# hasindu2008/cornetto

Hardware: AMD Instinct MI355X
Metric: Gbases/s scanned (telowin+sdust+boringbits) (higher is better)
Workload: dtype u8/u16 integer

## Files before the change

cornetto_amd/csrc/cov.hip:

```cpp
#include <algorithm>
#include <cmath>

#include "common.hpp"
#include "scan.hpp"
#include "tiles.hpp"
#include "ivlmerge.hpp"
#include "internal.hpp"

namespace {

constexpr int CB_THREADS = 256;
#ifndef CN_CB_PARTS
#define CN_CB_PARTS 2
#endif
constexpr int CB_PARTS = CN_CB_PARTS;
constexpr int CB_MAX_INC_LDS = 128;

struct CbArgs {
    const uint16_t *depth, *mq;
    const int64_t *ctg_off;
    const int32_t *ctg_len;
    const int2 *tiles;
    int32_t inc, r;
    uint2 *pre;
    uint2 *head;
    int64_t n_tiles;
    const int4 *tmeta;
    uint2 *tile_tot32;
    ulonglong2 *tile_tot64;
};

typedef unsigned short cb_us2 __attribute__((ext_vector_type(2)));
__device__ __forceinline__ uint32_t add_u16x2(uint32_t acc, uint32_t pair)
{
    const cb_us2 ones = {1, 1};
    return __builtin_amdgcn_udot2(__builtin_bit_cast(cb_us2, pair), ones, acc, false);
}

typedef unsigned int cb_u4 __attribute__((ext_vector_type(4)));

template <bool STAGE, int INC, int NT = 1>
__global__ __launch_bounds__(CB_THREADS) void cov_blocks(CbArgs A)
{
    __builtin_amdgcn_s_setprio(CN_STREAM_PRIO);

    extern __shared__ __attribute__((aligned(16))) uint8_t smem[];
    __shared__ uint32_t wsum[2][CB_THREADS / 64];
    __shared__ unsigned long long wsum64[2][CB_THREADS / 64];

    const int t = threadIdx.x;
    const int inc = INC ? INC : A.inc, r = A.r;
    constexpr int PBc = CB_THREADS / CB_PARTS;
    constexpr int NVIc = INC ? (PBc * INC / 8 + CB_THREADS - 1) / CB_THREADS : 4;
    cb_u4 pre_all[NT][2][CB_PARTS][NVIc];
    if (STAGE && INC) {
#pragma unroll
        for (int ti = 0; ti < NT; ++ti) {
            const int64_t tix = (int64_t)blockIdx.x * NT + ti;
            if (tix >= A.n_tiles) continue;
            int2 tl;
            int ln;
            int64_t of;
            if (A.tmeta) {
                const int4 m0 = A.tmeta[2 * tix], m1 = A.tmeta[2 * tix + 1];
                tl = make_int2(m0.x, m0.y); ln = m0.z; of = (int64_t)(((unsigned long long)(uint32_t)m1.y << 32) | (uint32_t)m1.x);
            } else {
                tl = A.tiles[tix]; ln = A.ctg_len[tl.x]; of = A.ctg_off[tl.x];
            }
            const int64_t e0l = (int64_t)tl.y * inc;
            const int nvec = PBc * inc / 8;
#pragma unroll
            for (int which = 0; which < 2; ++which)
#pragma unroll
                for (int part = 0; part < CB_PARTS; ++part) {
                    const int64_t pe0 = e0l + (int64_t)part * PBc * inc;
                    const int64_t left = ((int64_t)ln - pe0) * 2;
                    const uint32_t nrec = left <= 0 ? 0u : (uint32_t)(left < (int64_t)nvec * 16 ? (left + 15) & ~15LL : (int64_t)nvec * 16);
                    const __amdgpu_buffer_rsrc_t rs = __builtin_amdgcn_make_buffer_rsrc((void *)((which ? A.mq : A.depth) + of + pe0), 0, (int)nrec, 0x00020000);
#pragma unroll
                    for (int k = 0; k < NVIc; ++k) pre_all[ti][which][part][k] = __builtin_amdgcn_raw_buffer_load_b128(rs, (t + k * CB_THREADS) * 16, 0, 0);
                }
        }
    }
#pragma unroll
  for (int ti = 0; ti < NT; ++ti) {
    const int64_t tix = (int64_t)blockIdx.x * NT + ti;
    if (tix >= A.n_tiles) break;
    if (ti) __syncthreads();
    int2 tile;
    int len;
    int64_t off;
    if (A.tmeta) {
        const int4 m0 = A.tmeta[2 * tix], m1 = A.tmeta[2 * tix + 1];
        tile = make_int2(m0.x, m0.y); len = m0.z; off = (int64_t)(((unsigned long long)(uint32_t)m1.y << 32) | (uint32_t)m1.x);
    } else {
        tile = A.tiles[tix]; len = A.ctg_len[tile.x]; off = A.ctg_off[tile.x];
    }
    const int64_t e0 = (int64_t)tile.y * inc;
    const int64_t p0 = e0 + (int64_t)t * inc;

    uint32_t fd = 0, fq = 0, hd = 0, hq = 0;
    unsigned long long xd = 0, xq = 0;
    if (STAGE) {
        uint16_t *sv = reinterpret_cast<uint16_t *>(smem);
        constexpr int PB = CB_THREADS / CB_PARTS;
        const int nvec = PB * inc / 8;
        const int base = (t % PB) * inc;
        const int nval = p0 >= len ? 0 : (int)(len - p0 < inc ? len - p0 : inc);
        const int nh = r < nval ? r : nval;
        constexpr int NVI = NVIc;
        auto &pre = pre_all[ti];
#pragma unroll
        for (int which = 0; which < 2; ++which) {
#pragma unroll
            for (int part = 0; part < CB_PARTS; ++part) {
                const int64_t pe0 = e0 + (int64_t)part * PB * inc;
                const int64_t left = ((int64_t)len - pe0) * 2;
                const uint32_t nrec = left <= 0 ? 0u : (uint32_t)(left < (int64_t)nvec * 16 ? (left + 15) & ~15LL : (int64_t)nvec * 16);
                const __amdgpu_buffer_rsrc_t rs = __builtin_amdgcn_make_buffer_rsrc((void *)((which ? A.mq : A.depth) + off + pe0), 0, (int)nrec, 0x00020000);
                if (which | part) __syncthreads();
                constexpr int NV = 4;
                if (INC) {
#pragma unroll
                    for (int k = 0; k < NVI; ++k) {
                        const int v = t + k * CB_THREADS;
                        if (v < nvec) reinterpret_cast<cb_u4 *>(sv)[v] = pre[which][part][k];
                    }
                } else
                for (int v0 = t; v0 < nvec; v0 += NV * CB_THREADS) {
                    cb_u4 a[NV];
#pragma unroll
                    for (int k = 0; k < NV; ++k) a[k] = __builtin_amdgcn_raw_buffer_load_b128(rs, (v0 + k * CB_THREADS) * 16, 0, 0);
#pragma unroll
                    for (int k = 0; k < NV; ++k) {
                        const int v = v0 + k * CB_THREADS;
                        if (v < nvec) reinterpret_cast<cb_u4 *>(sv)[v] = a[k];
                    }
                }
                __syncthreads();
                if (t / PB == part) {
                    uint32_t f = 0, hh = 0;
                    if (INC && (INC & 1) == 0 && nval == inc) {
                        const uint32_t *wd = reinterpret_cast<const uint32_t *>(sv + base);
#pragma unroll
                        for (int i = 0; i < (INC ? INC : 2) / 2; ++i) f = add_u16x2(f, wd[i]);
                    } else if (nval == inc && (inc & 1) == 0) {
                        const uint32_t *wd = reinterpret_cast<const uint32_t *>(sv + base);
                        for (int i = 0; i < inc / 2; ++i) f = add_u16x2(f, wd[i]);
                    } else {
#pragma clang loop vectorize(disable) unroll(disable)
                        for (int i = 0; i < nval; ++i) f += sv[base + i];
                    }
#pragma clang loop vectorize(disable) unroll(disable)
                    for (int i = 0; i < nh; ++i) hh += sv[base + i];
// ... 169 lines not shown
        if (k % 3 == 2 && k + 1 < NR) __builtin_amdgcn_sched_barrier(0);
    }

    if (lane == 0) {
        wsum[0][wv] = cd[NR];
        wsum[1][wv] = cq[NR];
    }
    __syncthreads();
    const bool front = (uint32_t)(lane & 3) < wv;
    const uint32_t wd = wsum[0][lane & 3], wq = wsum[1][lane & 3];
    uint32_t fd = front ? wd : 0u, fq = front ? wq : 0u;
    fd += (uint32_t)__builtin_amdgcn_update_dpp(0, (int)fd, 0xB1, 0xF, 0xF, true);
    fq += (uint32_t)__builtin_amdgcn_update_dpp(0, (int)fq, 0xB1, 0xF, 0xF, true);
    fd += (uint32_t)__builtin_amdgcn_update_dpp(0, (int)fd, 0x4E, 0xF, 0xF, true);
    fq += (uint32_t)__builtin_amdgcn_update_dpp(0, (int)fq, 0x4E, 0xF, 0xF, true);
    const __amdgpu_buffer_rsrc_t rso = __builtin_amdgcn_make_buffer_rsrc((void *)(A.pre + (size_t)tix * CB_THREADS + wv * 64), 0, 64 * (int)sizeof(uint2), 0x00020000);
#pragma unroll
    for (int k = 0; k < NR; ++k) {
        const cb_u2 o = {od[k] + fd + cd[k], oq[k] + fq + cq[k]};
        __builtin_amdgcn_raw_buffer_store_b64(o, rso, (int)ooff[k], 0, 0);
    }
    if (wv == CB_THREADS / 64 - 1 && lane == 0) {
        A.tile_tot32[tix] = make_uint2(cd[NR] + fd, cq[NR] + fq);
        ulonglong2 x;
        x.x = cd[NR] + fd;
        x.y = cq[NR] + fq;
        A.tile_tot64[tix] = x;
    }
}

__global__ __launch_bounds__(256) void cov_total64(const ulonglong2 *tot64, int64_t n, unsigned long long *grand )
{
    __shared__ unsigned long long sa[4], sb[4];
    unsigned long long a = 0, b = 0;
    for (int64_t i = (int64_t)blockIdx.x * 256 + threadIdx.x; i < n; i += (int64_t)gridDim.x * 256) {
        const ulonglong2 v = tot64[i];
        a += v.x;
        b += v.y;
    }
#pragma unroll
    for (int d = 32; d >= 1; d >>= 1) {
        a += ((unsigned long long)__shfl_xor((unsigned)(a >> 32), d) << 32) | __shfl_xor((unsigned)a, d);
        b += ((unsigned long long)__shfl_xor((unsigned)(b >> 32), d) << 32) | __shfl_xor((unsigned)b, d);
    }
    if ((threadIdx.x & 63) == 0) {
        sa[threadIdx.x >> 6] = a;
        sb[threadIdx.x >> 6] = b;
    }
    __syncthreads();
    if (threadIdx.x == 0) {
        atomicAdd(&grand[0], sa[0] + sa[1] + sa[2] + sa[3]);
        atomicAdd(&grand[1], sb[0] + sb[1] + sb[2] + sb[3]);
    }
}

struct CwArgs {
    const uint2 *pre, *head;
    const uint32_t *toff_d, *toff_q;
    const int64_t *blk_off;
    const int32_t *ctg_len;
    const int32_t *n_reg;
    const int2 *tiles;
    int32_t w, inc, q, r;
    uint32_t w_magic, w_shift;
    int32_t mode;
    int32_t lo, hi, edge, min_len;
    double low_mq;
    cornetto_reg_t *regs;
    cornetto_regrec_t *sel;
    cornetto_regpk_t *pk;
    uint2 *tile_res;
};

__device__ __forceinline__ uint2 cw_prefix(const CwArgs &A, int64_t x)
{
    const uint2 b = A.pre[x];
    return make_uint2(b.x + A.toff_d[x >> 8], b.y + A.toff_q[x >> 8]);
}

__global__ __launch_bounds__(256) void cov_windows(CwArgs A)
{
    __builtin_amdgcn_s_setprio(CN_STREAM_PRIO);

    __shared__ uint32_t wcnt[4];
    const int t = threadIdx.x;
    const int2 tile = A.tiles[blockIdx.x];
    const int ctg = tile.x;
    const int len = A.ctg_len[ctg];
    const int j = tile.y + t;
    bool valid = j < A.n_reg[ctg];
    int st = 0, end = 0, depth = 0, mq = 0;
    bool sel = false;
    if (valid) {
        st = j * A.inc;
        end = st + A.w;
        if (end > len) end = len;
        const int64_t a = A.blk_off[ctg] + j;
        uint32_t sd = 0, sq = 0;
        if (A.q > 0) {
            const uint2 hi = cw_prefix(A, a + A.q - 1);
            uint2 lo = make_uint2(0, 0);
            if (a > 0) lo = cw_prefix(A, a - 1);
            sd = hi.x - lo.x;
            sq = hi.y - lo.y;
        }
        if (A.r) {
            const uint2 hb = A.head[a + A.q];
            sd += hb.x;
            sq += hb.y;
        }
        if (end - st == A.w && A.w_magic && (int32_t)(sd | sq) >= 0) {
            depth = (int32_t)(__umulhi(sd, A.w_magic) >> A.w_shift);
            mq = (int32_t)(__umulhi(sq, A.w_magic) >> A.w_shift);
        } else {
            depth = (int32_t)sd / (end - st);
            mq = (int32_t)sq / (end - st);
        }
        if (A.mode == 0) {
            A.regs[j] = cornetto_reg_t{st, end, depth, mq};
        } else {
            bool fun = depth < A.lo || depth > A.hi;
            if (!fun && !(A.low_mq <= 1.0 && depth > 0 && mq >= depth)) fun = ((double)mq / (double)depth) < A.low_mq;
            if (A.mode == 1) sel = len >= A.min_len && fun;
            else sel = len > A.min_len && st > A.edge && end < len - A.edge && !fun;
        }
    }
    if (A.mode == 0) return;
    const unsigned long long bal = __ballot(sel);
    const int lane = t & 63, wv = t >> 6;
    if (lane == 0) wcnt[wv] = (uint32_t)__popcll(bal);
    __syncthreads();
    uint32_t pre = 0, tot = 0;
#pragma unroll
    for (int i = 0; i < 4; ++i) {
        if (i < wv) pre += wcnt[i];
        tot += wcnt[i];
    }
    if (t == 0) A.tile_res[blockIdx.x] = make_uint2(blockIdx.x * 256u, tot);
    if (sel) {
        const size_t idx = (size_t)blockIdx.x * 256u + pre + __popcll(bal & ((1ull << lane) - 1ull));
        if (A.pk) A.pk[idx] = cornetto_regpk_t{st, (uint16_t)depth, (uint16_t)mq};
        else A.sel[idx] = cornetto_regrec_t{ctg, st, end, depth, mq};
    }
}

__global__ void cov_ctg_first(const uint32_t *ooff, const int32_t *first_tile, int32_t n_ctg, uint32_t n_tiles, const unsigned long long *total, uint32_t *out)
{
    const int32_t i = (int32_t)(blockIdx.x * blockDim.x + threadIdx.x);
    if (i >= n_ctg) return;
    const uint32_t t = (uint32_t)first_tile[i];
    out[i] = t < n_tiles ? ooff[t] : (uint32_t)*total;
}

template <int INTS>
__global__ __launch_bounds__(256) void cov_order(const int32_t *raw, const uint2 *tres, const uint32_t *ooff, int64_t n_tiles, int32_t *dst, const unsigned long long *total,
                                                 uint32_t cap)
{
    const int64_t t = (int64_t)blockIdx.x * 4 + (threadIdx.x >> 6);
    if (t >= n_tiles) return;
    if (*total > cap) return;
    const uint2 r = tres[t];
    const int32_t *src = raw + (size_t)r.x * INTS;
    int32_t *d = dst + (size_t)ooff[t] * INTS;
    const uint32_t nint = r.y * (uint32_t)INTS;
    for (uint32_t i = threadIdx.x & 63; i < nint; i += 64) d[i] = src[i];
}

__global__ __launch_bounds__(256) void cov_order_expand(const cornetto_regpk_t *raw, const uint2 *tres, const uint32_t *ooff, int64_t n_tiles, cornetto_regrec_t *dst,
                                                        const unsigned long long *total, uint32_t cap, const int2 *tiles, const int32_t *ctg_len, int32_t w)
{
    const int64_t t = (int64_t)blockIdx.x * 4 + (threadIdx.x >> 6);
    if (t >= n_tiles) return;
    if (*total > cap) return;
    const uint2 r = tres[t];
    const int32_t ctg = tiles[t].x, len = ctg_len[ctg];
    const cornetto_regpk_t *src = raw + r.x;
    cornetto_regrec_t *d = dst + ooff[t];
    for (uint32_t i = threadIdx.x & 63; i < r.y; i += 64) {
        const cornetto_regpk_t p = src[i];
        const int64_t e = (int64_t)p.st + w;
        d[i] = cornetto_regrec_t{ctg, p.st, e > len ? len : (int32_t)e, (int32_t)p.depth, (int32_t)p.mq_depth};
    }
}

int32_t n_reg_host(int32_t length, int32_t w, int32_t inc)
{
    int32_t n = (length - w + inc - 1) / inc + 1;
    return n < 1 ? 1 : n;
}

int32_t regs_assert_host(int32_t length, int32_t w, int32_t inc)
{
    const int64_t st = (int64_t)(n_reg_host(length, w, inc) - 1) * inc;
    int64_t end = st + w;
    if (end > length) end = length;
    if (!(st < end)) return 353;
    return end == length ? 0 : 368;
}

}

extern "C" {

int32_t cornetto_n_reg(int32_t length, int32_t window_size, int32_t window_inc)
{
    if (window_inc <= 0) return 0;
    return n_reg_host(length, window_size, window_inc);
}

int32_t cornetto_regs_assert(int32_t length, int32_t window_size, int32_t window_inc)
{
    if (window_inc <= 0) return 353;
    return regs_assert_host(length, window_size, window_inc);
}

int32_t cornetto_cov_threshold(float factor, int32_t mean)
{
    return (int32_t)round(factor * mean);
}

int cornetto_cov_prepare(cornetto_accel_t *h, cornetto_cov_t *c, int32_t w, int32_t inc, uint64_t sums[3])
{
    if (!h || !c || !sums) return cn_fail(h, CORNETTO_E_ARG, "cov_prepare: bad argument");
    CN_HIP(h, hipSetDevice(h->device));
    cn_timing_begin(h);
    const int rc = cn_cov_prepare_impl(h, c, w, inc, sums);
    if (rc == CORNETTO_OK) cn_timing_end(h);
    return rc;
}

}

struct CwTileFill {
    int2 *out;
    __device__ void operator()(int64_t t, int ci, int64_t j) const { out[t] = make_int2(ci, (int)(j * 256)); }
};
struct CbTileFill {
    int2 *tiles;
    int4 *tmeta;
    const int32_t *len;
    const int64_t *off;
    __device__ void operator()(int64_t t, int ci, int64_t j) const
    {
        const int b = (int)(j * CB_THREADS);
        const unsigned long long o = (unsigned long long)off[ci];
        tiles[t] = make_int2(ci, b);
        tmeta[2 * t] = make_int4(ci, b, len[ci], 0);
        tmeta[2 * t + 1] = make_int4((int)(uint32_t)o, (int)(uint32_t)(o >> 32), 0, 0);
    }
};

int cn_cov_prepare_impl(cornetto_accel_t *h, cornetto_cov_t *c, int32_t w, int32_t inc, uint64_t sums[3])
{
    if (inc < 1) return cn_fail(h, CORNETTO_E_UNSUPPORTED, "cov_prepare: needs window_inc >= 1 (got -i %d: the reference divides by it)", inc);
    for (int32_t i = 0; i < c->n; ++i) {
        const int32_t line = c->len[i] < 1 ? 0 : regs_assert_host(c->len[i], w, inc);
        if (line)
            return cn_fail(h, CORNETTO_E_ASSERT, "src/boringbits_main.c:%d: get_regs: Assertion `%s' failed. (contig %d of length %d, -w %d -i %d)", line,
                           line == 353 ? "st<end" : "end == length", i, c->len[i], w, inc);
    }
    const int32_t q = w / inc, r = w % inc;
    sums[0] = sums[1] = 0;
    sums[2] = (uint64_t)c->total;
    CN_TRACE("cov_prepare: enter");
    if (c->w != w || c->inc != inc || !c->d_blk) {
        struct Invalidate {
            cornetto_cov_t *c;
            bool keep = false;
            ~Invalidate() { if (!keep) c->w = c->inc = -1; }
        } built{c};
        c->w = w;
        c->inc = inc;
        c->cw_mode = -1;
        c->blk_off.assign(c->n + 1, 0);
        c->n_reg.assign(c->n, 0);
        for (int32_t i = 0; i < c->n; ++i) {
            if (c->len[i] < 1) return cn_fail(h, CORNETTO_E_ARG, "cov_prepare: contig %d is empty (a bedgraph cannot produce that)", i);
            c->n_reg[i] = n_reg_host(c->len[i], w, inc);
            c->blk_off[i + 1] = c->blk_off[i] + cn_align_up((int64_t)c->n_reg[i] + q + 1, CB_THREADS);
        }
        c->n_blk = c->blk_off[c->n];
        const int64_t ntl = cntiles::prefix(h, c->cb_pref, c->n, [&](int32_t i) { return (c->blk_off[i + 1] - c->blk_off[i]) / CB_THREADS; });
        if (ntl < 0) return cn_fail(h, CORNETTO_E_NOMEM, "cov_prepare: device allocation failed");
        c->n_cb_tiles = ntl;
        if (c->d_blk) { (void)hipFree(c->d_blk); c->d_blk = nullptr; }
        if (c->d_blk_off) { (void)hipFree(c->d_blk_off); c->d_blk_off = nullptr; }
        if (c->d_cb_tiles) { (void)hipFree(c->d_cb_tiles); c->d_cb_tiles = nullptr; }
        if (c->d_cb_tmeta) { (void)hipFree(c->d_cb_tmeta); c->d_cb_tmeta = nullptr; }
        if (c->d_n_reg) { (void)hipFree(c->d_n_reg); c->d_n_reg = nullptr; }
        const size_t nt = (size_t)ntl;
        if (nt == 0) { built.keep = true; return CORNETTO_OK; }
        if (cn_obj_malloc(h, (void **)&c->d_blk, (size_t)c->n_blk * sizeof(uint4) + 2 * nt * sizeof(uint32_t)) != hipSuccess ||
            cn_obj_malloc(h, (void **)&c->d_blk_off, (size_t)(c->n + 1) * 8) != hipSuccess ||
            cn_obj_malloc(h, (void **)&c->d_cb_tiles, nt * sizeof(int2)) != hipSuccess ||
            cn_obj_malloc(h, (void **)&c->d_cb_tmeta, 2 * nt * sizeof(int4)) != hipSuccess ||
            cn_obj_malloc(h, (void **)&c->d_n_reg, (size_t)c->n * 4) != hipSuccess)
            return cn_fail(h, CORNETTO_E_NOMEM, "cov_prepare: device allocation failed");
        cntiles::fill<<<dim3((unsigned)((nt + 255) / 256)), dim3(256), 0, h->stream>>>(c->cb_pref.dev, c->n, ntl, CbTileFill{c->d_cb_tiles, c->d_cb_tmeta, c->d_len, c->d_off});
        CN_HIP(h, hipGetLastError());
        CN_HIP(h, hipMemcpyAsync(c->d_blk_off, c->blk_off.data(), (size_t)(c->n + 1) * 8, hipMemcpyHostToDevice, h->stream));
        CN_HIP(h, hipMemcpyAsync(c->d_n_reg, c->n_reg.data(), (size_t)c->n * 4, hipMemcpyHostToDevice, h->stream));
        built.keep = true;
    }
    CN_TRACE("cov_prepare: tables");
    const size_t nt = (size_t)c->n_cb_tiles;
    if (nt == 0) return CORNETTO_OK;
    uint2 *d_t32 = (uint2 *)cn_ws(h, WS_CB_T32, nt * sizeof(uint2));
    ulonglong2 *d_t64 = (ulonglong2 *)cn_ws(h, WS_CB_T64, nt * sizeof(ulonglong2));
    unsigned long long *d_grand = (unsigned long long *)cn_ws(h, WS_CB_GRAND, 16);
    unsigned long long *p_grand = (unsigned long long *)cn_pin(h, PIN_SMALL, 64);
    if (!d_t32 || !d_t64 || !d_grand || !p_grand) return cn_fail(h, CORNETTO_E_NOMEM, "cov_prepare: workspace allocation failed");
    uint2 *d_pre = reinterpret_cast<uint2 *>(c->d_blk), *d_head = d_pre + c->n_blk;
    uint32_t *d_toff_d = reinterpret_cast<uint32_t *>(d_head + c->n_blk), *d_toff_q = d_toff_d + nt;
    CN_TRACE("cov_prepare: workspaces");
    CN_HIP(h, hipMemsetAsync(d_grand, 0, 16, h->stream));
    static const int cb_tmeta = CN_DEV_INT("CORNETTO_COV_TMETA", 1);
    CbArgs A{c->d_depth, c->d_mq, c->d_off, c->d_len, c->d_cb_tiles, inc, r, d_pre, d_head, (int64_t)nt, cb_tmeta ? c->d_cb_tmeta : nullptr, d_t32, d_t64};
    if (inc <= CB_MAX_INC_LDS) {
        const size_t lds = (size_t)CB_THREADS / CB_PARTS * inc * sizeof(uint16_t);
        static_assert(CB_THREADS / CB_PARTS * 50 / 8 <= 4 * CB_THREADS, "cov_blocks<true, INC>: at most 4 vectors per thread and part");
        if (A.inc == 50 && r == 0 && A.tmeta && !CN_DEV_INT("CORNETTO_COV_BLOCKS_STAGE", 0)) {
            CN_LAUNCH(h, "cov_blocks", cov_blocks_scan<50><<<dim3((unsigned)nt), dim3(CB_THREADS), 0, h->stream>>>(A, CbsPattern<50>{}.masks()));
        } else if (A.inc == 50) {
            static const int cb_nt = CN_DEV_INT("CORNETTO_COV_TILES", 1);
            if (cb_nt == 2) {
                CN_HIP(h, hipFuncSetAttribute(reinterpret_cast<const void *>(&cov_blocks<true, 50, 2>), hipFuncAttributeMaxDynamicSharedMemorySize, (int)lds));
                CN_LAUNCH(h, "cov_blocks", cov_blocks<true, 50, 2><<<dim3((unsigned)((nt + 1) / 2)), dim3(CB_THREADS), lds, h->stream>>>(A));
            } else {
                CN_HIP(h, hipFuncSetAttribute(reinterpret_cast<const void *>(&cov_blocks<true, 50>), hipFuncAttributeMaxDynamicSharedMemorySize, (int)lds));
                CN_LAUNCH(h, "cov_blocks", cov_blocks<true, 50><<<dim3((unsigned)nt), dim3(CB_THREADS), lds, h->stream>>>(A));
            }
        } else {
            CN_HIP(h, hipFuncSetAttribute(reinterpret_cast<const void *>(&cov_blocks<true, 0>), hipFuncAttributeMaxDynamicSharedMemorySize, (int)lds));
            CN_LAUNCH(h, "cov_blocks", cov_blocks<true, 0><<<dim3((unsigned)nt), dim3(CB_THREADS), lds, h->stream>>>(A));
        }
    } else {
        CN_LAUNCH(h, "cov_blocks", cov_blocks<false, 0><<<dim3((unsigned)nt), dim3(CB_THREADS), 0, h->stream>>>(A));
    }
    {
        uint32_t *const outs[2] = {d_toff_d, d_toff_q};
        CN_TRY(cnscan::exclusive_u32_multi(h, "cov_tilescan", reinterpret_cast<const uint32_t *>(d_t32), (int64_t)nt, 2, 2, outs, nullptr));
    }
    const unsigned nb64 = (unsigned)std::min<size_t>(1024, (nt + 255) / 256);
    CN_LAUNCH(h, "cov_total64", cov_total64<<<dim3(nb64), dim3(256), 0, h->stream>>>(d_t64, (int64_t)nt, d_grand));
    CN_HIP(h, hipMemcpyAsync(p_grand, d_grand, 16, hipMemcpyDeviceToHost, h->stream));
    CN_TRACE("cov_prepare: queued");
    CN_HIP(h, hipStreamSynchronize(h->stream));
    CN_TRACE("cov_prepare: done");
    sums[0] = p_grand[0] - c->sum_corr[0];
    sums[1] = p_grand[1] - c->sum_corr[1];
    c->sums[0] = sums[0]; c->sums[1] = sums[1]; c->sums[2] = (uint64_t)c->total;
    return CORNETTO_OK;
}

extern "C" {

static int64_t cov_est_key(const cornetto_cov_t *c, int mode, int32_t lo, int32_t hi, float low_mq, int32_t edge, int32_t min_len)
{
    uint32_t qb;
    memcpy(&qb, &low_mq, 4);
    uint64_t k = 1469598103934665603ull;
    for (uint64_t v : {(uint64_t)(uint32_t)mode, (uint64_t)(uint32_t)lo, (uint64_t)(uint32_t)hi, (uint64_t)qb, (uint64_t)(uint32_t)edge, (uint64_t)(uint32_t)min_len,
                       (uint64_t)(uint32_t)c->w, (uint64_t)(uint32_t)c->inc})
        k = (k ^ v) * 1099511628211ull;
    return (int64_t)(k >> 1);
}

static int cov_run_windows(cornetto_accel_t *h, cornetto_cov_t *c, int32_t only_ctg, int mode, int32_t lo, int32_t hi,
                           float low_mq, int32_t edge, int32_t min_len, cornetto_reg_t *regs_host, cornetto_regrec_t **recs,
                           int64_t *n_recs, bool keep_on_device = false, cornetto_regpk_t **pk_out = nullptr, int64_t **ctg_first = nullptr,
                           CnCovSpec *spec = nullptr)
{
    const bool packed = pk_out != nullptr || spec != nullptr;
    CN_TRACE("cov_select: enter");
    const int64_t est_key = cov_est_key(c, mode, lo, hi, low_mq, edge, min_len);
    if (spec) {
        spec->queued = false;
        if (c->cw_est_key != est_key || c->cw_est_cnt < 0) return CORNETTO_OK;
    }
    const size_t rec_bytes = packed ? sizeof(cornetto_regpk_t) : sizeof(cornetto_regrec_t);
    if (!c->d_blk) return cn_fail(h, CORNETTO_E_ARG, "cov: cornetto_cov_prepare() has not been called");
    const int32_t w = c->w, inc = c->inc, q = w / inc, r = w % inc;
    const bool raw_packed = w <= 32768;
    if (packed && !raw_packed) return cn_fail(h, CORNETTO_E_UNSUPPORTED, "cov_select_packed: window size %d > 32768 (a wrapped sum's mean does not fit 16 bits)", w);
    const size_t raw_bytes = raw_packed ? sizeof(cornetto_regpk_t) : sizeof(cornetto_regrec_t);
    if (c->cw_mode != mode || c->cw_min_len != min_len || c->cw_only != only_ctg) {
        const int64_t ntl = cntiles::prefix(h, c->cw_pref, c->n, [&](int32_t i) -> int64_t {
            if (only_ctg >= 0 && i != only_ctg) return 0;
            if (mode == 1 && !(c->len[i] >= min_len)) return 0;
            if (mode == 2 && !(c->len[i] > min_len)) return 0;
            return ((int64_t)c->n_reg[i] + 255) / 256;
        });
        if (ntl < 0) return cn_fail(h, CORNETTO_E_NOMEM, "cov: device allocation failed");
        if (c->d_cw_tiles) { (void)hipFree(c->d_cw_tiles); c->d_cw_tiles = nullptr; }
        if (c->d_cw_first) { (void)hipFree(c->d_cw_first); c->d_cw_first = nullptr; }
        c->n_cw_tiles = ntl;
        if (ntl > 0) {
            c->cw_first.resize((size_t)c->n + 1);
            for (int32_t i = 0; i <= c->n; ++i) c->cw_first[i] = (int32_t)c->cw_pref.host[i];
            if (cn_obj_malloc(h, (void **)&c->d_cw_tiles, (size_t)ntl * sizeof(int2)) != hipSuccess || cn_obj_malloc(h, (void **)&c->d_cw_first, ((size_t)c->n + 1) * 4) != hipSuccess)
                return cn_fail(h, CORNETTO_E_NOMEM, "cov: device allocation failed");
            cntiles::fill<<<dim3((unsigned)((ntl + 255) / 256)), dim3(256), 0, h->stream>>>(c->cw_pref.dev, c->n, ntl, CwTileFill{c->d_cw_tiles});
            CN_HIP(h, hipGetLastError());
            CN_HIP(h, hipMemcpyAsync(c->d_cw_first, c->cw_first.data(), (size_t)c->n * 4, hipMemcpyHostToDevice, h->stream));
        }
        c->cw_mode = mode;
        c->cw_min_len = min_len;
        c->cw_only = only_ctg;
    }
    const size_t nt = (size_t)c->n_cw_tiles;
    if (nt == 0) return CORNETTO_OK;
    const size_t nt_blk = (size_t)c->n_cb_tiles;
    const uint2 *d_pre = reinterpret_cast<const uint2 *>(c->d_blk), *d_head = d_pre + c->n_blk;
    const uint32_t *d_toff_d = reinterpret_cast<const uint32_t *>(d_head + c->n_blk), *d_toff_q = d_toff_d + nt_blk;
    unsigned long long *d_cnt = (unsigned long long *)cn_ws(h, WS_CW_CNT, 16);
    uint2 *d_tres = (uint2 *)cn_ws(h, WS_CW_TRES, nt * 12);
    unsigned long long *p_cnt = spec ? spec->p_cnt : (unsigned long long *)cn_pin(h, PIN_SMALL, 64);
    if (!d_cnt || !d_tres || !p_cnt) return cn_fail(h, CORNETTO_E_NOMEM, "cov: workspace allocation failed");
    uint32_t *d_ooff = reinterpret_cast<uint32_t *>(d_tres + nt);
    CwArgs A{};
    A.pre = d_pre; A.head = d_head; A.toff_d = d_toff_d; A.toff_q = d_toff_q; A.blk_off = c->d_blk_off; A.ctg_len = c->d_len; A.n_reg = c->d_n_reg;
    A.tiles = c->d_cw_tiles; A.w = w; A.inc = inc; A.q = q; A.r = r; A.mode = mode; A.lo = lo; A.hi = hi; A.edge = edge;
    if (w >= 2) {
        int L = 0;
        while ((1ll << L) < (long long)w) ++L;
        A.w_magic = (uint32_t)(((1ull << (31 + L)) / (unsigned long long)w) + 1ull);
        A.w_shift = (uint32_t)(L - 1);
    }
    A.min_len = min_len; A.low_mq = (double)low_mq;
    A.tile_res = d_tres;
    if (mode == 0) {
        const size_t nr = (size_t)c->n_reg[only_ctg];
        cornetto_reg_t *d_regs = (cornetto_reg_t *)cn_ws(h, WS_CW_REGS, nr * sizeof(cornetto_reg_t));
        if (!d_regs) return cn_fail(h, CORNETTO_E_NOMEM, "cov: workspace allocation failed");
        A.regs = d_regs;
        CN_LAUNCH(h, "cov_windows", cov_windows<<<dim3((unsigned)nt), dim3(256), 0, h->stream>>>(A));
        CN_HIP(h, hipMemcpyAsync(regs_host, d_regs, nr * sizeof(cornetto_reg_t), hipMemcpyDeviceToHost, h->stream));
        CN_HIP(h, hipStreamSynchronize(h->stream));
        return CORNETTO_OK;
    }
    const size_t n_raw = nt * 256;
    if (n_raw > 0xffffff00ull) return cn_fail(h, CORNETTO_E_UNSUPPORTED, "cov: %zu window tiles", nt);
    size_t cap = std::max<size_t>(1 << 16, nt * 256 / 8);
    if (h->dev[WS_CW_SEL].bytes > n_raw * raw_bytes) cap = std::max(cap, (h->dev[WS_CW_SEL].bytes - n_raw * raw_bytes) / rec_bytes);
    unsigned long long cnt = 0;
    cornetto_regrec_t *d_raw = nullptr, *d_dst = nullptr;
    uint32_t *p_cf = nullptr, *d_cf = nullptr;
    if (packed) {
        p_cf = (uint32_t *)cn_pin(h, PIN_CW, ((size_t)c->n + 1) * 4);
        d_cf = (uint32_t *)cn_ws(h, WS_CW_CF, ((size_t)c->n + 1) * 4);
        if (!p_cf || !d_cf) return cn_fail(h, CORNETTO_E_NOMEM, "cov_select: allocation failed");
    }
    CN_TRACE("cov_select: tables + small workspaces");
    for (int attempt = 0; attempt < 2; ++attempt) {
        cap = std::min<size_t>(cap, 0x7fffffff);
        d_raw = (cornetto_regrec_t *)cn_ws(h, WS_CW_SEL, n_raw * raw_bytes + cap * rec_bytes);
        if (!d_raw) return cn_fail(h, CORNETTO_E_NOMEM, "cov: workspace allocation of %zu bytes failed", n_raw * raw_bytes + cap * rec_bytes);
        d_dst = reinterpret_cast<cornetto_regrec_t *>(reinterpret_cast<uint8_t *>(d_raw) + n_raw * raw_bytes);
        A.sel = d_raw;
        A.pk = raw_packed ? reinterpret_cast<cornetto_regpk_t *>(d_raw) : nullptr;
        CN_LAUNCH(h, "cov_windows", cov_windows<<<dim3((unsigned)nt), dim3(256), 0, h->stream>>>(A));
        CN_TRY(cnscan::exclusive_u32(h, "cov_order", reinterpret_cast<const uint32_t *>(d_tres) + 1, (int64_t)nt, 2, d_ooff, d_cnt));
        const unsigned nb = (unsigned)((nt + 3) / 4);
        hipEvent_t ea = cn_event(h), eb = cn_event(h);
        (void)hipEventRecord(ea, h->stream);
        if (packed) cov_order<2><<<dim3(nb), dim3(256), 0, h->stream>>>(reinterpret_cast<const int32_t *>(d_raw), d_tres, d_ooff, (int64_t)nt, reinterpret_cast<int32_t *>(d_dst), d_cnt, (uint32_t)cap);
        else if (raw_packed) cov_order_expand<<<dim3(nb), dim3(256), 0, h->stream>>>(reinterpret_cast<const cornetto_regpk_t *>(d_raw), d_tres, d_ooff, (int64_t)nt, d_dst, d_cnt, (uint32_t)cap, c->d_cw_tiles, c->d_len, w);
        else cov_order<5><<<dim3(nb), dim3(256), 0, h->stream>>>(reinterpret_cast<const int32_t *>(d_raw), d_tres, d_ooff, (int64_t)nt, reinterpret_cast<int32_t *>(d_dst), d_cnt, (uint32_t)cap);
        (void)hipEventRecord(eb, h->stream);
        h->recs.push_back(cornetto_accel::Rec{"cov_order", ea, eb});
        if (hipGetLastError() != hipSuccess) return cn_fail(h, CORNETTO_E_HIP, "cov_select: ordering failed");
        if (packed) {
            cov_ctg_first<<<dim3((unsigned)((c->n + 255) / 256)), dim3(256), 0, h->stream>>>(d_ooff, c->d_cw_first, c->n, (uint32_t)nt, d_cnt, d_cf);
            if (hipGetLastError() != hipSuccess || hipMemcpyAsync(p_cf, d_cf, (size_t)c->n * 4, hipMemcpyDeviceToHost, h->stream) != hipSuccess)
                return cn_fail(h, CORNETTO_E_HIP, "cov_select: first records of the contigs failed");
        }
        CN_HIP(h, hipMemcpyAsync(p_cnt, d_cnt, 8, hipMemcpyDeviceToHost, h->stream));
        if (spec) {
            size_t n_copy = std::min<size_t>(cap, (size_t)c->cw_est_cnt + (size_t)c->cw_est_cnt / 16 + 1024);
            if (const int f = CN_DEV_INT("CORNETTO_STEP_EST_FORCE", 0)) n_copy = std::min<size_t>(cap, (size_t)std::max(1, f));
            cornetto_regpk_t *o = (cornetto_regpk_t *)cn_result_alloc(n_copy * rec_bytes);
            if (!o) return cn_fail(h, CORNETTO_E_NOMEM, "cov_select: host allocation failed");
            if (cn_result_d2h(h, o, d_dst, n_copy * rec_bytes) != hipSuccess) {
                cn_result_quiesce(h);
                cornetto_free(o);
                return cn_fail(h, CORNETTO_E_HIP, "cov_select: copy back failed");
            }
            spec->queued = true; spec->o = o; spec->n_copy = n_copy; spec->cap = cap; spec->p_cf = p_cf; spec->key = est_key;
            return CORNETTO_OK;
        }
        CN_HIP(h, hipStreamSynchronize(h->stream));
        cnt = p_cnt[0];
        if (cnt <= cap) break;
        if (attempt == 1 || cnt > 0x7fffffffull) return cn_fail(h, CORNETTO_E_UNSUPPORTED, "cov: %llu selected windows", cnt);
        cap = (size_t)cnt;
    }
    CN_TRACE("cov_select: kernels done, count known");
    cornetto_regrec_t *o = keep_on_device ? d_dst : (cornetto_regrec_t *)cn_result_alloc((cnt ? cnt : 1) * rec_bytes);
    CN_TRACE("cov_select: result block");
    if (!o) return cn_fail(h, CORNETTO_E_NOMEM, "cov_select: host allocation failed");
    if (cnt) {
        if (!keep_on_device && (cn_result_d2h(h, o, d_dst, (size_t)cnt * rec_bytes) != hipSuccess || (!h->lazy && hipStreamSynchronize(h->stream) != hipSuccess))) {
            cn_result_quiesce(h);
            cornetto_free(o);
            return cn_fail(h, CORNETTO_E_HIP, "cov_select: copy back failed");
        }
        if (packed) {
            int64_t *cf = (int64_t *)malloc(((size_t)c->n + 1) * sizeof(int64_t));
            if (!cf) { cn_result_quiesce(h); cornetto_free(o); return cn_fail(h, CORNETTO_E_NOMEM, "cov_select: host allocation failed"); }
            for (int32_t i = 0; i < c->n; ++i) cf[i] = (int64_t)p_cf[i];
            cf[c->n] = (int64_t)cnt;
            *ctg_first = cf;
        }
    } else if (packed) {
        int64_t *cf = (int64_t *)calloc((size_t)c->n + 1, sizeof(int64_t));
        if (!cf) { if (!keep_on_device) cornetto_free(o); return cn_fail(h, CORNETTO_E_NOMEM, "cov_select: host allocation failed"); }
        *ctg_first = cf;
    }
    if (packed) {
        *pk_out = reinterpret_cast<cornetto_regpk_t *>(o);
        c->cw_est_key = est_key;
        c->cw_est_cnt = (int64_t)cnt;
    } else {
        *recs = o;
    }
    *n_recs = (int64_t)cnt;
    return CORNETTO_OK;
}

int cornetto_cov_regs(cornetto_accel_t *h, const cornetto_cov_t *c, int32_t ctg, cornetto_reg_t *regs)
{
    if (!h || !c || !regs || ctg < 0 || ctg >= c->n) return cn_fail(h, CORNETTO_E_ARG, "cov_regs: bad argument");
    CN_HIP(h, hipSetDevice(h->device));
    cn_timing_begin(h);
    int rc = cov_run_windows(h, const_cast<cornetto_cov_t *>(c), ctg, 0, 0, 0, 0.f, 0, 0, regs, nullptr, nullptr);
    cn_timing_end(h);
    return rc;
}

int cornetto_cov_select(cornetto_accel_t *h, const cornetto_cov_t *c, int32_t lo, int32_t hi, float low_mq, int32_t edge_len,
                        int32_t min_ctg_len, int boring, cornetto_regrec_t **recs, int64_t *n_recs)
{
    if (!h || !c || !recs || !n_recs) return cn_fail(h, CORNETTO_E_ARG, "cov_select: bad argument");
    *recs = nullptr;
    *n_recs = 0;
    CN_HIP(h, hipSetDevice(h->device));
    cn_timing_begin(h);
    int rc = cov_run_windows(h, const_cast<cornetto_cov_t *>(c), -1, boring ? 2 : 1, lo, hi, low_mq, edge_len, min_ctg_len, nullptr, recs, n_recs);
    cn_timing_end(h);
    if (rc == CORNETTO_OK && !*recs) {
        *recs = (cornetto_regrec_t *)malloc(sizeof(cornetto_regrec_t));
        if (!*recs) return cn_fail(h, CORNETTO_E_NOMEM, "cov_select: host allocation failed");
    }
    return rc;
}

int cornetto_cov_select_packed(cornetto_accel_t *h, const cornetto_cov_t *c, int32_t lo, int32_t hi, float low_mq, int32_t edge_len,
                               int32_t min_ctg_len, int boring, cornetto_regpk_t **recs, int64_t *n_recs, int64_t **ctg_first)
{
    if (!h || !c || !recs || !n_recs || !ctg_first) return cn_fail(h, CORNETTO_E_ARG, "cov_select_packed: bad argument");
    CN_HIP(h, hipSetDevice(h->device));
    cn_timing_begin(h);
    const int rc = cn_cov_select_packed_impl(h, const_cast<cornetto_cov_t *>(c), lo, hi, low_mq, edge_len, min_ctg_len, boring, recs, n_recs, ctg_first);
    cn_timing_end(h);
    return rc;
}

}

int cn_cov_spec_queue(cornetto_accel_t *h, cornetto_cov_t *c, int32_t lo, int32_t hi, float low_mq, int32_t edge_len, int32_t min_ctg_len, int boring,
                      unsigned long long *p_cnt, CnCovSpec *S)
{
    S->p_cnt = p_cnt;
    return cov_run_windows(h, c, -1, boring ? 2 : 1, lo, hi, low_mq, edge_len, min_ctg_len, nullptr, nullptr, nullptr, false, nullptr, nullptr, S);
}

int cn_cov_spec_finish(cornetto_accel_t *h, cornetto_cov_t *c, CnCovSpec *S, cornetto_regpk_t **recs, int64_t *n_recs, int64_t **ctg_first)
{
    if (!S->queued) return 1;
    S->queued = false;
    const unsigned long long cnt = S->p_cnt[0];
    int64_t *cf = cnt <= S->n_copy ? (int64_t *)malloc(((size_t)c->n + 1) * sizeof(int64_t)) : nullptr;
    if (!cf) {
        cn_result_quiesce(h);
        cornetto_free(S->o);
        S->o = nullptr;
        c->cw_est_key = -1;
        return cnt <= S->n_copy ? cn_fail(h, CORNETTO_E_NOMEM, "cov_select: host allocation failed") : 1;
    }
    for (int32_t i = 0; i < c->n; ++i) cf[i] = (int64_t)S->p_cf[i];
    cf[c->n] = (int64_t)cnt;
    *recs = S->o;
    *n_recs = (int64_t)cnt;
    *ctg_first = cf;
    S->o = nullptr;
    c->cw_est_key = S->key;
    c->cw_est_cnt = (int64_t)cnt;
    return CORNETTO_OK;
}

int cn_cov_select_packed_impl(cornetto_accel_t *h, cornetto_cov_t *c, int32_t lo, int32_t hi, float low_mq, int32_t edge_len, int32_t min_ctg_len, int boring,
                              cornetto_regpk_t **recs, int64_t *n_recs, int64_t **ctg_first)
{
    *recs = nullptr;
    *n_recs = 0;
    *ctg_first = nullptr;
    int rc = cov_run_windows(h, c, -1, boring ? 2 : 1, lo, hi, low_mq, edge_len, min_ctg_len, nullptr, nullptr, n_recs, false, recs, ctg_first);
    if (rc == CORNETTO_OK && !*recs) {
        *recs = (cornetto_regpk_t *)malloc(sizeof(cornetto_regpk_t));
        if (!*ctg_first) *ctg_first = (int64_t *)calloc((size_t)c->n + 1, sizeof(int64_t));
        if (!*recs || !*ctg_first) return cn_fail(h, CORNETTO_E_NOMEM, "cov_select_packed: host allocation failed");
    }
    return rc;
}

extern "C" {

namespace {
__global__ void cov_rec_spans(const cornetto_regrec_t *r, int64_t n, cornetto_ivl_t *out)
{
    const int64_t i = (int64_t)blockIdx.x * blockDim.x + threadIdx.x;
    if (i < n) out[i] = cornetto_ivl_t{r[i].ctg, r[i].st, r[i].end};
}
}
// ... 47 lines not shown
```

cornetto_amd/csrc/scan.hpp:

```cpp
#pragma once
#include "common.hpp"
#include "wave.hpp"

namespace cnscan {
namespace {

constexpr int SC_THREADS = 256;
constexpr int SC_ITEMS = 16;
constexpr int SC_TILE = SC_THREADS * SC_ITEMS;

template <typename T, int THREADS>
__device__ __forceinline__ T block_excl(T s, T &total)
{
    __shared__ T wtot[THREADS / 64];
    const int lane = threadIdx.x & 63, wv = threadIdx.x >> 6;
    const T inc = cnwave::wave_incl(s, lane);
    if (lane == 63) wtot[wv] = inc;
    __syncthreads();
    T pre = inc - s;
    total = 0;
#pragma unroll
    for (int w = 0; w < THREADS / 64; ++w) {
        if (w < wv) pre += wtot[w];
        total += wtot[w];
    }
    return pre;
}

template <typename T, int ITEMS>
__device__ __forceinline__ T tile_excl(const T *in, int64_t base, int64_t n, int stride, T (&v)[ITEMS], T &total)
{
    T s = 0;
#pragma unroll
    for (int k = 0; k < ITEMS; ++k) {
        const int64_t i = base + k;
        v[k] = i < n ? in[i * stride] : (T)0;
        s += v[k];
    }
    return block_excl<T, SC_THREADS>(s, total);
}

template <typename T, int ITEMS>
__device__ __forceinline__ void tile_write(T *out, int64_t base, int64_t n, T pre, const T (&v)[ITEMS])
{
#pragma unroll
    for (int k = 0; k < ITEMS; ++k) {
        const int64_t i = base + k;
        if (i < n) out[i] = pre;
        pre += v[k];
    }
}

__device__ __forceinline__ uint32_t lookback_excl(unsigned long long *st, int64_t stride, int64_t tile, uint32_t epoch, uint32_t own, int lane)
{
    const unsigned long long tag = (unsigned long long)(epoch & 0x3FFFFFFFu) << 32;
    uint32_t excl = 0;
    if (tile > 0) {
        if (lane == 0) __hip_atomic_store(&st[tile * stride], (1ull << 62) | tag | own, __ATOMIC_RELAXED, __HIP_MEMORY_SCOPE_AGENT);
        for (int64_t pos = tile - 1;; pos -= 64) {
            const int64_t idx = pos - lane;
            unsigned long long x;
            for (;;) {
                x = idx >= 0 ? __hip_atomic_load(&st[idx * stride], __ATOMIC_RELAXED, __HIP_MEMORY_SCOPE_AGENT) : ((2ull << 62) | tag);
                const bool ready = (x >> 62) != 0 && (x & (0x3FFFFFFFull << 32)) == tag;
                if (__builtin_amdgcn_ballot_w64(!ready) == 0) break;
                __builtin_amdgcn_s_sleep(1);
            }
            const unsigned long long incl = __builtin_amdgcn_ballot_w64((x >> 62) == 2);
            const uint32_t val = (uint32_t)x;
            if (incl) {
                const int first = __builtin_ctzll(incl);
                excl += cnwave::wave_sum(lane <= first ? val : 0u);
                break;
            }
            excl += cnwave::wave_sum(val);
        }
    }
    if (lane == 0) __hip_atomic_store(&st[tile * stride], (2ull << 62) | tag | (excl + own), __ATOMIC_RELAXED, __HIP_MEMORY_SCOPE_AGENT);
    return excl;
}

struct Outs4 {
    uint32_t *o[4];
};
struct LbArgs {
    const uint32_t *in;
    int64_t n, np;
    int stride, m;
    Outs4 outs;
    unsigned long long *state;
    uint32_t *ticket;
    uint32_t ticket_base, epoch;
    unsigned long long *total;
};

__global__ __launch_bounds__(SC_THREADS) void scan_lookback(LbArgs A)
{
    __shared__ uint32_t s_gid, s_excl;
    const int t = threadIdx.x, lane = t & 63, wv = t >> 6;
    if (t == 0) s_gid = atomicAdd(A.ticket, 1u) - A.ticket_base;
    __syncthreads();
    const int64_t gid = s_gid;
    if (gid >= (int64_t)A.m * A.np) return;
    const int q = (int)(gid / A.np);
    const int64_t tile = gid - (int64_t)q * A.np;
    const int64_t base = tile * SC_TILE + (int64_t)t * SC_ITEMS;
    uint32_t v[SC_ITEMS], bt;
    uint32_t pre = tile_excl(A.in + q, base, A.n, A.stride, v, bt);
    if (wv == 0) {
        const uint32_t excl = lookback_excl(A.state + (int64_t)q * A.np, 1, tile, A.epoch, bt, lane);
        if (lane == 0) {
            s_excl = excl;
            if (A.total && tile == A.np - 1) A.total[q] = (unsigned long long)excl + bt;
        }
    }
    __syncthreads();
    pre += s_excl;
    tile_write(A.outs.o[q], base, A.n, pre, v);
}

static inline int exclusive_u32_multi(cornetto_accel_t *h, const char *name, const uint32_t *in, int64_t n, int stride, int m, uint32_t *const *outs,
                                      unsigned long long *d_total)
{
    if (n <= 0 || m <= 0) return CORNETTO_OK;
    if (m > 4) m = 4;
    Outs4 o{};
    for (int q = 0; q < m; ++q) o.o[q] = outs[q];
    const int64_t np = (n + SC_TILE - 1) / SC_TILE;
    const size_t need = 64 + (size_t)m * (size_t)np * 8;
    const bool fresh = h->dev[WS_SCAN].bytes < need || h->scan_epoch >= 0x3FFFFFFFu;
    uint8_t *ws = (uint8_t *)cn_ws(h, WS_SCAN, need);
    if (!ws) return cn_fail(h, CORNETTO_E_NOMEM, "scan: workspace allocation failed");
    const int rc = [&]() -> int {
        if (fresh) {
            CN_HIP(h, hipMemsetAsync(ws, 0, h->dev[WS_SCAN].bytes, h->stream));
            h->scan_tickets = 0;
            h->scan_epoch = 0;
        }
        const uint32_t epoch = h->scan_epoch + 1;
        LbArgs A{in, n, np, stride, m, o, reinterpret_cast<unsigned long long *>(ws + 64), reinterpret_cast<uint32_t *>(ws), h->scan_tickets, epoch, d_total};
        CN_LAUNCH(h, name, scan_lookback<<<dim3((unsigned)(m * np)), dim3(SC_THREADS), 0, h->stream>>>(A));
        h->scan_epoch = epoch;
        h->scan_tickets += (uint32_t)(m * np);
        return CORNETTO_OK;
    }();
    if (rc != CORNETTO_OK) h->dev[WS_SCAN].bytes = 0;
    return rc;
}

static inline int exclusive_u32(cornetto_accel_t *h, const char *name, const uint32_t *in, int64_t n, int stride, uint32_t *out, unsigned long long *d_total)
{
    return exclusive_u32_multi(h, name, in, n, stride, 1, &out, d_total);
}

}
}
```

Measured before the change: 515.4.

## Fuse tile-count scan into cov_order compaction with decoupled lookback

```diff
diff --git a/cornetto_amd/csrc/cov.hip b/cornetto_amd/csrc/cov.hip
--- a/cornetto_amd/csrc/cov.hip
+++ b/cornetto_amd/csrc/cov.hip
@@ -1,5 +1,6 @@
 #include <algorithm>
 #include <cmath>
+#include <type_traits>
 
 #include "common.hpp"
 #include "scan.hpp"
@@ -475,34 +476,83 @@
     out[i] = t < n_tiles ? ooff[t] : (uint32_t)*total;
 }
 
-template <int INTS>
-__global__ __launch_bounds__(256) void cov_order(const int32_t *raw, const uint2 *tres, const uint32_t *ooff, int64_t n_tiles, int32_t *dst, const unsigned long long *total,
-                                                 uint32_t cap)
-{
-    const int64_t t = (int64_t)blockIdx.x * 4 + (threadIdx.x >> 6);
-    if (t >= n_tiles) return;
-    if (*total > cap) return;
-    const uint2 r = tres[t];
-    const int32_t *src = raw + (size_t)r.x * INTS;
-    int32_t *d = dst + (size_t)ooff[t] * INTS;
-    const uint32_t nint = r.y * (uint32_t)INTS;
-    for (uint32_t i = threadIdx.x & 63; i < nint; i += 64) d[i] = src[i];
-}
-
-__global__ __launch_bounds__(256) void cov_order_expand(const cornetto_regpk_t *raw, const uint2 *tres, const uint32_t *ooff, int64_t n_tiles, cornetto_regrec_t *dst,
-                                                        const unsigned long long *total, uint32_t cap, const int2 *tiles, const int32_t *ctg_len, int32_t w)
-{
-    const int64_t t = (int64_t)blockIdx.x * 4 + (threadIdx.x >> 6);
-    if (t >= n_tiles) return;
-    if (*total > cap) return;
-    const uint2 r = tres[t];
-    const int32_t ctg = tiles[t].x, len = ctg_len[ctg];
-    const cornetto_regpk_t *src = raw + r.x;
-    cornetto_regrec_t *d = dst + ooff[t];
-    for (uint32_t i = threadIdx.x & 63; i < r.y; i += 64) {
-        const cornetto_regpk_t p = src[i];
-        const int64_t e = (int64_t)p.st + w;
-        d[i] = cornetto_regrec_t{ctg, p.st, e > len ? len : (int32_t)e, (int32_t)p.depth, (int32_t)p.mq_depth};
+constexpr int CO_TILES = 256;
+constexpr int CO_U = 8;
+struct CoArgs {
+    const void *raw;
+    const uint2 *tres;
+    int64_t n_tiles;
+    void *dst;
+    uint32_t cap;
+    unsigned long long *state;
+    uint32_t *ticket;
+    uint32_t ticket_base, epoch;
+    uint32_t *ooff;
+    unsigned long long *total;
+    const int2 *tiles;
+    const int32_t *ctg_len;
+    int32_t w;
+};
+
+template <typename RAW, typename OUT>
+__global__ __launch_bounds__(256) void cov_order(CoArgs A)
+{
+    constexpr bool EXPAND = !std::is_same<RAW, OUT>::value;
+    __shared__ uint32_t s_gid, s_excl, s_cnt[CO_TILES], s_off[CO_TILES];
+    const int t = threadIdx.x, lane = t & 63, wv = t >> 6;
+    if (t == 0) s_gid = atomicAdd(A.ticket, 1u) - A.ticket_base;
+    __syncthreads();
+    const int64_t g = s_gid, t0 = g * CO_TILES;
+    if (t0 >= A.n_tiles) return;
+    const bool mine = t < CO_TILES && t0 + t < A.n_tiles;
+    const uint32_t c = mine ? A.tres[t0 + t].y : 0u;
+    uint32_t tot;
+    uint32_t pre = cnscan::block_excl<uint32_t, 256>(c, tot);
+    if (wv == 0) {
+        const uint32_t excl = cnscan::lookback_excl(A.state, 1, g, A.epoch, tot, lane);
+        if (lane == 0) {
+            s_excl = excl;
+            if (t0 + CO_TILES >= A.n_tiles) *A.total = (unsigned long long)excl + tot;
+        }
+    }
+    __syncthreads();
+    pre += s_excl;
+    if (mine) A.ooff[t0 + t] = pre;
+    if (t < CO_TILES) {
+        s_off[t] = pre;
+        s_cnt[t] = !mine || pre >= A.cap ? 0u : min(c, A.cap - pre);
+    }
+    __syncthreads();
+    const RAW *__restrict__ raw = static_cast<const RAW *>(A.raw) + t0 * 256;
+    OUT *__restrict__ dst = static_cast<OUT *>(A.dst);
+    auto put = [&](int k, uint32_t i, const RAW &v) {
+        if constexpr (EXPAND) {
+            const int32_t ctg = A.tiles[t0 + k].x, len = A.ctg_len[ctg];
+            const int64_t e = (int64_t)v.st + A.w;
+            dst[s_off[k] + i] = OUT{ctg, v.st, e > len ? len : (int32_t)e, (int32_t)v.depth, (int32_t)v.mq_depth};
+        } else {
+            dst[s_off[k] + i] = v;
+        }
+    };
+    constexpr int U = sizeof(RAW) > 8 ? 1 : CO_U;
+    for (int k0 = wv; k0 < CO_TILES; k0 += 4 * U) {
+        RAW v[U];
+#pragma unroll
+        for (int u = 0; u < U; ++u) {
+            const int k = k0 + 4 * u;
+            if (k < CO_TILES && (uint32_t)lane < s_cnt[k]) v[u] = raw[(size_t)k * 256 + lane];
+        }
+#pragma unroll
+        for (int u = 0; u < U; ++u) {
+            const int k = k0 + 4 * u;
+            if (k < CO_TILES && (uint32_t)lane < s_cnt[k]) put(k, lane, v[u]);
+        }
+#pragma unroll
+        for (int u = 0; u < U; ++u) {
+            const int k = k0 + 4 * u;
+            if (k < CO_TILES)
+                for (uint32_t i = lane + 64; i < s_cnt[k]; i += 64) put(k, i, raw[(size_t)k * 256 + i]);
+        }
     }
 }
 
@@ -783,16 +833,15 @@
         A.sel = d_raw;
         A.pk = raw_packed ? reinterpret_cast<cornetto_regpk_t *>(d_raw) : nullptr;
         CN_LAUNCH(h, "cov_windows", cov_windows<<<dim3((unsigned)nt), dim3(256), 0, h->stream>>>(A));
-        CN_TRY(cnscan::exclusive_u32(h, "cov_order", reinterpret_cast<const uint32_t *>(d_tres) + 1, (int64_t)nt, 2, d_ooff, d_cnt));
-        const unsigned nb = (unsigned)((nt + 3) / 4);
-        hipEvent_t ea = cn_event(h), eb = cn_event(h);
-        (void)hipEventRecord(ea, h->stream);
-        if (packed) cov_order<2><<<dim3(nb), dim3(256), 0, h->stream>>>(reinterpret_cast<const int32_t *>(d_raw), d_tres, d_ooff, (int64_t)nt, reinterpret_cast<int32_t *>(d_dst), d_cnt, (uint32_t)cap);
-        else if (raw_packed) cov_order_expand<<<dim3(nb), dim3(256), 0, h->stream>>>(reinterpret_cast<const cornetto_regpk_t *>(d_raw), d_tres, d_ooff, (int64_t)nt, d_dst, d_cnt, (uint32_t)cap, c->d_cw_tiles, c->d_len, w);
-        else cov_order<5><<<dim3(nb), dim3(256), 0, h->stream>>>(reinterpret_cast<const int32_t *>(d_raw), d_tres, d_ooff, (int64_t)nt, reinterpret_cast<int32_t *>(d_dst), d_cnt, (uint32_t)cap);
-        (void)hipEventRecord(eb, h->stream);
-        h->recs.push_back(cornetto_accel::Rec{"cov_order", ea, eb});
-        if (hipGetLastError() != hipSuccess) return cn_fail(h, CORNETTO_E_HIP, "cov_select: ordering failed");
+        CoArgs O{d_raw, d_tres, (int64_t)nt, d_dst, (uint32_t)cap, nullptr, nullptr, 0, 0, d_ooff, d_cnt, c->d_cw_tiles, c->d_len, w};
+        const unsigned nb = (unsigned)((nt + CO_TILES - 1) / CO_TILES);
+        CN_TRY(cnscan::with_lookback(h, (int64_t)nb, [&](const cnscan::Lookback &L) -> int {
+            O.state = L.state; O.ticket = L.ticket; O.ticket_base = L.ticket_base; O.epoch = L.epoch;
+            if (packed) CN_LAUNCH(h, "cov_order", cov_order<cornetto_regpk_t, cornetto_regpk_t><<<dim3(nb), dim3(256), 0, h->stream>>>(O));
+            else if (raw_packed) CN_LAUNCH(h, "cov_order", cov_order<cornetto_regpk_t, cornetto_regrec_t><<<dim3(nb), dim3(256), 0, h->stream>>>(O));
+            else CN_LAUNCH(h, "cov_order", cov_order<cornetto_regrec_t, cornetto_regrec_t><<<dim3(nb), dim3(256), 0, h->stream>>>(O));
+            return CORNETTO_OK;
+        }));
         if (packed) {
             cov_ctg_first<<<dim3((unsigned)((c->n + 255) / 256)), dim3(256), 0, h->stream>>>(d_ooff, c->d_cw_first, c->n, (uint32_t)nt, d_cnt, d_cf);
             if (hipGetLastError() != hipSuccess || hipMemcpyAsync(p_cf, d_cf, (size_t)c->n * 4, hipMemcpyDeviceToHost, h->stream) != hipSuccess)
diff --git a/cornetto_amd/csrc/scan.hpp b/cornetto_amd/csrc/scan.hpp
--- a/cornetto_amd/csrc/scan.hpp
+++ b/cornetto_amd/csrc/scan.hpp
@@ -119,15 +119,16 @@
     tile_write(A.outs.o[q], base, A.n, pre, v);
 }
 
-static inline int exclusive_u32_multi(cornetto_accel_t *h, const char *name, const uint32_t *in, int64_t n, int stride, int m, uint32_t *const *outs,
-                                      unsigned long long *d_total)
+struct Lookback {
+    unsigned long long *state;
+    uint32_t *ticket;
+    uint32_t ticket_base, epoch;
+};
+
+template <typename F>
+static inline int with_lookback(cornetto_accel_t *h, int64_t n_tickets, F &&launch)
 {
-    if (n <= 0 || m <= 0) return CORNETTO_OK;
-    if (m > 4) m = 4;
-    Outs4 o{};
-    for (int q = 0; q < m; ++q) o.o[q] = outs[q];
-    const int64_t np = (n + SC_TILE - 1) / SC_TILE;
-    const size_t need = 64 + (size_t)m * (size_t)np * 8;
+    const size_t need = 64 + (size_t)n_tickets * 8;
     const bool fresh = h->dev[WS_SCAN].bytes < need || h->scan_epoch >= 0x3FFFFFFFu;
     uint8_t *ws = (uint8_t *)cn_ws(h, WS_SCAN, need);
     if (!ws) return cn_fail(h, CORNETTO_E_NOMEM, "scan: workspace allocation failed");
@@ -138,14 +139,28 @@
             h->scan_epoch = 0;
         }
         const uint32_t epoch = h->scan_epoch + 1;
-        LbArgs A{in, n, np, stride, m, o, reinterpret_cast<unsigned long long *>(ws + 64), reinterpret_cast<uint32_t *>(ws), h->scan_tickets, epoch, d_total};
-        CN_LAUNCH(h, name, scan_lookback<<<dim3((unsigned)(m * np)), dim3(SC_THREADS), 0, h->stream>>>(A));
+        CN_TRY(launch(Lookback{reinterpret_cast<unsigned long long *>(ws + 64), reinterpret_cast<uint32_t *>(ws), h->scan_tickets, epoch}));
         h->scan_epoch = epoch;
-        h->scan_tickets += (uint32_t)(m * np);
+        h->scan_tickets += (uint32_t)n_tickets;
         return CORNETTO_OK;
     }();
     if (rc != CORNETTO_OK) h->dev[WS_SCAN].bytes = 0;
     return rc;
+}
+
+static inline int exclusive_u32_multi(cornetto_accel_t *h, const char *name, const uint32_t *in, int64_t n, int stride, int m, uint32_t *const *outs,
+                                      unsigned long long *d_total)
+{
+    if (n <= 0 || m <= 0) return CORNETTO_OK;
+    if (m > 4) m = 4;
+    Outs4 o{};
+    for (int q = 0; q < m; ++q) o.o[q] = outs[q];
+    const int64_t np = (n + SC_TILE - 1) / SC_TILE;
+    return with_lookback(h, (int64_t)m * np, [&](const Lookback &L) -> int {
+        LbArgs A{in, n, np, stride, m, o, L.state, L.ticket, L.ticket_base, L.epoch, d_total};
+        CN_LAUNCH(h, name, scan_lookback<<<dim3((unsigned)(m * np)), dim3(SC_THREADS), 0, h->stream>>>(A));
+        return CORNETTO_OK;
+    });
 }
 
 static inline int exclusive_u32(cornetto_accel_t *h, const char *name, const uint32_t *in, int64_t n, int stride, uint32_t *out, unsigned long long *d_total)
```

New measurement: 503.2. 2.4% lower.
